# microsoft/XPretrain

Hardware: NVIDIA H100
Metric: video-text pairs/sec (12f x 224^2, 32 tok), CLIP-ViP ViT-B/16 fwd+InfoNCE+bwd (higher is better)
Workload: dtype bf16

## Files before the change

include/xpretrain_b200.h:

```cpp
#ifndef XPRETRAIN_B200_H
#define XPRETRAIN_B200_H

#include <stddef.h>
#include <stdint.h>

#ifdef __cplusplus
extern "C" {
#endif

#define XP_ABI_VERSION 1

int xp_version(void);
const char* xp_last_error(void);
int64_t xp_launch_count(void);
void xp_launch_count_reset(void);

enum { XP_ACT_NONE = 0, XP_ACT_QUICK_GELU = 1, XP_ACT_DQUICK_GELU = 2, XP_ACT_GELU_ERF = 3, XP_ACT_DGELU_ERF = 4 };
enum { XP_OUT_BF16 = 0, XP_OUT_F32 = 1, XP_OUT_F32_ATOMIC = 2 };

typedef struct XpGemm {
  const void* a;
  const void* b;
  void* c;
  const float* bias;
  const void* residual;
  void* aux;
  int64_t M, N, K;
  int64_t lda, ldb, ldc, ldr, ld_aux;
  int32_t a_layout, b_layout;
  int32_t act, out;
  int32_t splits;
  int32_t scale_cols;
  float alpha, col_scale;
  int64_t c_group, c_group_stride, r_group, r_group_stride;
  int32_t block_n;
  int32_t max_ctas;
  int32_t cta_pair;
  int32_t reserved;
} XpGemm;

int xp_gemm(const XpGemm* g, void* stream);

typedef struct XpRowMap {
  int64_t group, group_stride, ld;
  const int64_t* offsets;
} XpRowMap;

int xp_layernorm_fwd(const void* x, const XpRowMap* xmap, void* y, const XpRowMap* ymap, const float* gamma,
// ... 162 lines not shown
```

xpretrain_b200/_lib.py:

```python
from __future__ import annotations

import ctypes as C
import os

_HERE = os.path.dirname(os.path.abspath(__file__))
LIB_PATH = os.path.join(_HERE, "lib", "libxpretrain_b200.so")

c_void_p, c_int, c_i64, c_float = C.c_void_p, C.c_int32, C.c_int64, C.c_float


class XpGemm(C.Structure):
    _fields_ = [
        ("a", c_void_p), ("b", c_void_p), ("c", c_void_p), ("bias", c_void_p), ("residual", c_void_p), ("aux", c_void_p),
        ("M", c_i64), ("N", c_i64), ("K", c_i64),
        ("lda", c_i64), ("ldb", c_i64), ("ldc", c_i64), ("ldr", c_i64), ("ld_aux", c_i64),
        ("a_layout", c_int), ("b_layout", c_int), ("act", c_int), ("out", c_int),
        ("splits", c_int), ("scale_cols", c_int), ("alpha", c_float), ("col_scale", c_float),
        ("c_group", c_i64), ("c_group_stride", c_i64), ("r_group", c_i64), ("r_group_stride", c_i64),
        ("block_n", c_int), ("max_ctas", c_int), ("cta_pair", c_int), ("reserved", c_int),
    ]


class XpRowMap(C.Structure):
    _fields_ = [("group", c_i64), ("group_stride", c_i64), ("ld", c_i64), ("offsets", c_void_p)]
# ... 8 lines not shown

class XpDenseAttn(C.Structure):
    _fields_ = [("n_rows", c_i64), ("ld_qkv", c_i64), ("ld_out", c_i64), ("heads", c_int), ("n_seq", c_int),
                ("seq_len", c_int), ("reserved", c_int)]


class XpNceGather(C.Structure):
    _fields_ = [("vis_local", c_void_p), ("txt_local", c_void_p), ("peer_bufs", c_void_p), ("logit_scale", c_void_p),
                ("g_scaled", c_void_p), ("vis_hi", c_void_p), ("txt_hi", c_void_p), ("loss", c_void_p),
                ("d_logit_scale", c_void_p), ("workspace", c_void_p), ("rank", c_int), ("world", c_int), ("b", c_int),
                ("d", c_int), ("epoch", C.c_uint32), ("mode", c_int), ("ld_g", c_i64)]


class XpNceTerm(C.Structure):
    _fields_ = [("axis", c_int), ("members", c_int), ("excl_diag", c_int), ("target", c_int)]


class XpNceTerms(C.Structure):
    _fields_ = [("z", c_void_p * 3), ("g", c_void_p * 3), ("ld", c_i64 * 3), ("n", c_int * 3), ("n_mats", c_int),
                ("n_terms", c_int), ("term", XpNceTerm * 6), ("logit_scale", c_void_p), ("scale", c_float),
                ("loss", c_void_p), ("d_logit_scale", c_void_p), ("workspace", c_void_p)]


ACT_NONE, ACT_QUICK_GELU, ACT_DQUICK_GELU, ACT_GELU_ERF, ACT_DGELU_ERF = 0, 1, 2, 3, 4
OUT_BF16, OUT_F32, OUT_F32_ATOMIC = 0, 1, 2
DTYPE_F32, DTYPE_BF16, DTYPE_F16 = 0, 1, 2

P = C.POINTER
SIGNATURES = {
    "xp_version": (c_int, []),
    "xp_last_error": (C.c_char_p, []),
    "xp_launch_count": (c_i64, []),
    "xp_launch_count_reset": (None, []),
    "xp_gemm": (c_int, [P(XpGemm), c_void_p]),
    "xp_layernorm_fwd": (c_int, [c_void_p, P(XpRowMap), c_void_p, P(XpRowMap), c_void_p, c_void_p, c_void_p, c_void_p,
                                 c_i64, c_int, c_float, c_void_p]),
    "xp_layernorm_add_fwd": (c_int, [c_void_p, P(XpRowMap), c_int, c_void_p, P(XpRowMap), c_void_p, P(XpRowMap), c_void_p,
                                     P(XpRowMap), c_int, c_void_p, c_void_p, c_void_p, c_void_p, c_i64, c_int, c_float,
                                     c_void_p]),
    "xp_layernorm_bwd": (c_int, [c_void_p, P(XpRowMap), c_void_p, P(XpRowMap), c_int, c_void_p, c_void_p, c_void_p, c_void_p,
                                 P(XpRowMap), c_void_p, P(XpRowMap), c_void_p, c_void_p, c_void_p, c_i64, c_int, c_void_p]),
    "xp_l2norm_fwd": (c_int, [c_void_p, c_void_p, c_void_p, c_int, c_int, c_void_p]),
    "xp_l2norm_bwd": (c_int, [c_void_p, c_void_p, c_void_p, c_void_p, c_int, c_int, c_float, c_void_p]),
    "xp_frame_pool_fwd": (c_int, [c_void_p, c_void_p, c_void_p, c_void_p, c_int, c_int, c_int, c_void_p]),
    "xp_frame_pool_bwd": (c_int, [c_void_p, c_void_p, c_void_p, c_void_p, c_void_p, c_void_p, c_int, c_int, c_int,
                                  c_float, c_void_p]),
    "xp_colsum_bf16": (c_int, [c_void_p, c_i64, c_void_p, c_i64, c_int, c_float, c_void_p]),
    "xp_cast_f32_bf16": (c_int, [c_void_p, c_void_p, c_i64, c_void_p]),
    "xp_vip_patchify": (c_int, [c_void_p, c_int, c_void_p, c_i64, c_int, c_int, c_int, c_void_p]),
    "xp_vip_patchify_u8": (c_int, [c_void_p, c_void_p, c_i64, c_int, c_int, c_int, P(c_float), P(c_float), c_void_p]),
    "xp_vip_embed_tables": (c_int, [c_void_p, c_void_p, c_void_p, c_void_p, c_void_p, c_void_p, c_int, c_int, c_int,
                                    c_int, c_int, c_int, c_void_p]),
    "xp_vip_embed_bwd": (c_int, [c_void_p, c_void_p, c_void_p, c_void_p, c_void_p, c_void_p, c_int, c_int, c_int, c_int,
                                 c_int, c_int, c_void_p]),
    "xp_text_embed_fwd": (c_int, [c_void_p, c_void_p, c_void_p, c_void_p, c_int, c_int, c_int, c_int, c_void_p,
                                  c_void_p]),
    "xp_text_embed_bwd": (c_int, [c_void_p, c_void_p, c_void_p, c_void_p, c_int, c_int, c_int, c_int, c_void_p]),
    "xp_eos_offsets": (c_int, [c_void_p, c_void_p, c_void_p, c_int, c_int, c_int, c_void_p]),
    "xp_vip_attention_workspace_bytes": (c_i64, [c_int, c_int, c_int, c_int]),
    "xp_vip_attention_fwd": (c_int, [c_void_p, c_void_p, c_void_p, c_void_p, c_int, c_int, c_int, c_int, c_int, c_int,
                                     c_void_p]),
    "xp_vip_attention_bwd": (c_int, [c_void_p, c_void_p, c_void_p, c_void_p, c_void_p, c_void_p, c_int, c_int, c_int,
                                     c_int, c_int, c_int, c_float, c_void_p]),
    "xp_text_attention_fwd": (c_int, [c_void_p, c_void_p, c_void_p, c_void_p, c_int, c_int, c_int, c_int, c_void_p]),
    "xp_text_attention_bwd": (c_int, [c_void_p, c_void_p, c_void_p, c_void_p, c_int, c_int, c_int, c_int, c_float,
                                      c_void_p]),
# ... 59 lines not shown
```

xpretrain_b200/csrc/attn_wgmma.cuh:

```cuda
#pragma once
#include "ptx.cuh"
#include "mma_frag.cuh"

namespace xp {

constexpr int ATILE = 64;
constexpr int ATILE_BYTES = ATILE * 128;
constexpr int STREAM_THREADS = 384;

constexpr int stream_fwd_smem(int stages) { return (2 + 2 * stages) * ATILE_BYTES + 1024 + 64; }
constexpr int stream_kv_smem(int stages) { return (4 + 2 * stages) * ATILE_BYTES + stages * 2 * ATILE * 4 + 1024 + 64; }
constexpr int stream_q_smem(int stages) { return (4 + 2 * stages) * ATILE_BYTES + 1024 + 64; }

__device__ __forceinline__ uint64_t kdesc(uint32_t addr) { return make_smem_desc_sw128(addr, 16, 1024); }
__device__ __forceinline__ uint64_t mndesc(uint32_t addr) { return make_smem_desc_sw128(addr, 8192, 1024); }

__device__ __forceinline__ void acc_to_afrag(const float (&x)[32], uint32_t (&a)[4][4]) {
#pragma unroll
  for (int ks = 0; ks < 4; ++ks) {
    a[ks][0] = pack_bf16(x[8 * ks + 0], x[8 * ks + 1]);
    a[ks][1] = pack_bf16(x[8 * ks + 2], x[8 * ks + 3]);
    a[ks][2] = pack_bf16(x[8 * ks + 4], x[8 * ks + 5]);
    a[ks][3] = pack_bf16(x[8 * ks + 6], x[8 * ks + 7]);
  }
// ... 43 lines not shown
  for (int i = 0; i < 32; ++i) {
    const float pv = fast_exp2(fmaf(s[i], LOG2E, -mb[(i >> 1) & 1]));
    s[i] = pv;
    l_run[(i >> 1) & 1] += pv;
  }
  uint32_t ph[4][4], pl[4][4];
  acc_to_afrag(s, ph);
#pragma unroll
  for (int ks = 0; ks < 4; ++ks)
#pragma unroll
    for (int j = 0; j < 4; ++j)
      pl[ks][j] = pack_bf16(s[8 * ks + 2 * j] - bf16_lo(ph[ks][j]), s[8 * ks + 2 * j + 1] - bf16_hi(ph[ks][j]));
  wgmma_fence_regs(o);
  wgmma_fence();
#pragma unroll
  for (int ks = 0; ks < 4; ++ks) {
    const uint64_t vd = mndesc(sV + ks * 16 * 128);
    wgmma_m64n64k16_rs<1>(o, ph[ks], vd);
    wgmma_m64n64k16_rs<1>(o, pl[ks], vd);
  }
  wgmma_commit();
  wgmma_wait<0>();
  wgmma_fence_regs(o);
}

__device__ __forceinline__ void quad_sum(float (&l_run)[2]) {
#pragma unroll
  for (int r = 0; r < 2; ++r) {
    l_run[r] += __shfl_xor_sync(0xffffffffu, l_run[r], 1);
    l_run[r] += __shfl_xor_sync(0xffffffffu, l_run[r], 2);
  }
}

template <class Live>
__device__ __forceinline__ void kv_step(uint32_t sK, uint32_t sV, uint32_t sQ, uint32_t sdO, const float* s_lse,
                                        const float* s_delta, float (&dk)[32], float (&dv)[32], Live live) {
  const int lane = threadIdx.x & 31, k_lo = ((threadIdx.x >> 5) & 3) * 16 + (lane >> 2);
  float st[32], dpt[32];
#pragma unroll
  for (int i = 0; i < 32; ++i) st[i] = dpt[i] = 0.f;
  wgmma_fence_regs(st);
  wgmma_fence_regs(dpt);
  wgmma_fence();
#pragma unroll
  for (int ks = 0; ks < 4; ++ks) {
    wgmma_m64n64k16_ss<0, 0>(st, kdesc(sK + ks * 32), kdesc(sQ + ks * 32));
    wgmma_m64n64k16_ss<0, 0>(dpt, kdesc(sV + ks * 32), kdesc(sdO + ks * 32));
  }
  wgmma_commit();
  wgmma_wait<0>();
  wgmma_fence_regs(st);
  wgmma_fence_regs(dpt);
#pragma unroll
  for (int i = 0; i < 8; ++i)
#pragma unroll
    for (int e = 0; e < 4; ++e) {
      const int q = i * 8 + (lane & 3) * 2 + (e & 1);
      const float p = live(q, k_lo + (e >> 1) * 8) ? fast_exp2(fmaf(st[4 * i + e], LOG2E, -s_lse[q])) : 0.f;
      st[4 * i + e] = p;
      dpt[4 * i + e] = p * (dpt[4 * i + e] - s_delta[q]);
    }
  uint32_t ap[4][4], ad[4][4];
  acc_to_afrag(st, ap);
  acc_to_afrag(dpt, ad);
  wgmma_fence_regs(dv);
  wgmma_fence_regs(dk);
  wgmma_fence();
#pragma unroll
  for (int ks = 0; ks < 4; ++ks) {
    wgmma_m64n64k16_rs<1>(dv, ap[ks], mndesc(sdO + ks * 16 * 128));
    wgmma_m64n64k16_rs<1>(dk, ad[ks], mndesc(sQ + ks * 16 * 128));
  }
  wgmma_commit();
  wgmma_wait<0>();
  wgmma_fence_regs(dv);
  wgmma_fence_regs(dk);
}

template <class Live>
__device__ __forceinline__ void q_step(uint32_t sQ, uint32_t sdO, uint32_t sK, uint32_t sV, const float (&lse_r)[2],
                                       const float (&del_r)[2], float (&dq)[32], Live live) {
  const int lane = threadIdx.x & 31, q_lo = ((threadIdx.x >> 5) & 3) * 16 + (lane >> 2);
  float s[32], dp[32];
#pragma unroll
  for (int i = 0; i < 32; ++i) s[i] = dp[i] = 0.f;
  wgmma_fence_regs(s);
  wgmma_fence_regs(dp);
  wgmma_fence();
#pragma unroll
  for (int ks = 0; ks < 4; ++ks) {
    wgmma_m64n64k16_ss<0, 0>(s, kdesc(sQ + ks * 32), kdesc(sK + ks * 32));
    wgmma_m64n64k16_ss<0, 0>(dp, kdesc(sdO + ks * 32), kdesc(sV + ks * 32));
  }
  wgmma_commit();
  wgmma_wait<0>();
  wgmma_fence_regs(s);
  wgmma_fence_regs(dp);
#pragma unroll
  for (int i = 0; i < 8; ++i)
#pragma unroll
    for (int e = 0; e < 4; ++e) {
      const bool valid = live(q_lo + (e >> 1) * 8, i * 8 + (lane & 3) * 2 + (e & 1));
      const float p = valid ? fast_exp2(fmaf(s[4 * i + e], LOG2E, -lse_r[e >> 1])) : 0.f;
      dp[4 * i + e] = p * (dp[4 * i + e] - del_r[e >> 1]);
    }
  uint32_t ad[4][4];
  acc_to_afrag(dp, ad);
  wgmma_fence_regs(dq);
  wgmma_fence();
#pragma unroll
  for (int ks = 0; ks < 4; ++ks) wgmma_m64n64k16_rs<1>(dq, ad[ks], mndesc(sK + ks * 16 * 128));
  wgmma_commit();
  wgmma_wait<0>();
  wgmma_fence_regs(dq);
}

template <int STAGES>
__device__ __forceinline__ void init_ring(uint64_t* q_full, uint64_t* full, uint64_t* empty, uint32_t full_count,
                                          int nlive, const CUtensorMap* tm0, const CUtensorMap* tm1) {
  if (threadIdx.x == 0) {
    tma_prefetch_desc(tm0);
    tma_prefetch_desc(tm1);
    mbar_init(q_full, 1);
#pragma unroll
    for (int s = 0; s < STAGES; ++s) {
      mbar_init(&full[s], full_count);
      mbar_init(&empty[s], 4 * nlive);
    }
    fence_barrier_init();
  }
  __syncthreads();
}
__device__ __forceinline__ void release_stage(uint64_t* empty, int s) {
  __syncwarp();
  if ((threadIdx.x & 31) == 0) mbar_arrive(&empty[s]);
}

template <class P>
__device__ __forceinline__ void produce_kv_blocks(const P& p, const CUtensorMap* tm, uint8_t* sm, int ring,
                                                  uint64_t* full, uint64_t* empty) {
  for (int kb = 0; kb < p.ntiles(); ++kb) {
    const int s = kb % P::STAGES;
    mbar_wait_nocall(&empty[s], ((kb / P::STAGES) & 1) ^ 1);
    uint8_t* st = sm + (ring + 2 * s) * ATILE_BYTES;
// ... 187 lines not shown
```

xpretrain_b200/csrc/common.cu:

```cuda
#include "common.h"

#include <mutex>

#include "../../include/xpretrain_b200.h"

namespace xp {

static thread_local std::string t_error;
std::atomic<int64_t> g_launches{0};

void set_error(const std::string& msg) { t_error = msg; }
int fail(const std::string& msg) {
  t_error = msg;
  return -1;
}

int sm_count() {
  static int cached[64] = {0};
  int dev = 0;
  if (cudaGetDevice(&dev) != cudaSuccess || dev < 0 || dev >= 64) return 132;
  if (cached[dev] == 0) {
    int n = 0;
    if (cudaDeviceGetAttribute(&n, cudaDevAttrMultiProcessorCount, dev) != cudaSuccess || n <= 0) n = 132;
    cached[dev] = n;
  }
  return cached[dev];
}

typedef CUresult (*EncodeTiledFn)(CUtensorMap*, CUtensorMapDataType, cuuint32_t, void*, const cuuint64_t*,
                                  const cuuint64_t*, const cuuint32_t*, const cuuint32_t*, CUtensorMapInterleave,
                                  CUtensorMapSwizzle, CUtensorMapL2promotion, CUtensorMapFloatOOBfill);

static EncodeTiledFn encode_fn() {
  static EncodeTiledFn fn = nullptr;
  static std::once_flag once;
  std::call_once(once, [] {
    void* p = nullptr;
    cudaDriverEntryPointQueryResult q;
    if (cudaGetDriverEntryPoint("cuTensorMapEncodeTiled", &p, cudaEnableDefault, &q) == cudaSuccess &&
        q == cudaDriverEntryPointSuccess)
      fn = reinterpret_cast<EncodeTiledFn>(p);
  });
  return fn;
}

typedef CUresult (*CtxGetCurrentFn)(CUcontext*);
typedef CUresult (*CtxSetCurrentFn)(CUcontext);
typedef CUresult (*PointerGetAttributeFn)(void*, CUpointer_attribute, CUdeviceptr);

static void* driver_symbol(const char* name) {
  void* p = nullptr;
  cudaDriverEntryPointQueryResult q;
  if (cudaGetDriverEntryPoint(name, &p, cudaEnableDefault, &q) != cudaSuccess || q != cudaDriverEntryPointSuccess)
    return nullptr;
  return p;
}

int ensure_context(const void* device_ptr) {
  static thread_local bool bound = false;
// ... 38 lines not shown
  cuuint32_t estr[2] = {1, 1};
  CUresult r = fn(out, CU_TENSOR_MAP_DATA_TYPE_BFLOAT16, 2, const_cast<void*>(base), dims, strides, box, estr,
                  CU_TENSOR_MAP_INTERLEAVE_NONE, CU_TENSOR_MAP_SWIZZLE_128B, CU_TENSOR_MAP_L2_PROMOTION_L2_256B,
                  CU_TENSOR_MAP_FLOAT_OOB_FILL_NONE);
  if (r != CUDA_SUCCESS) return fail("cuTensorMapEncodeTiled failed with CUresult " + std::to_string(int(r)));
  return 0;
}

int make_tmap_bf16_3d(CUtensorMap* out, const void* base, uint64_t inner, uint64_t mid, uint64_t outer,
                      uint64_t row_stride, uint64_t mid_stride, uint32_t box_inner, uint32_t box_mid) {
  EncodeTiledFn fn = encode_fn();
  if (!fn) return fail("cuTensorMapEncodeTiled unavailable (no CUDA driver / no GPU): this library has no CPU path");
  if ((reinterpret_cast<uintptr_t>(base) & 15) != 0) return fail("tensor map: base pointer must be 16-byte aligned");
  if ((row_stride * 2) % 16 != 0 || (mid_stride * 2) % 16 != 0)
    return fail("tensor map: strides must be multiples of 8 bf16 elements");
  cuuint64_t dims[3] = {inner, mid, outer};
  cuuint64_t strides[2] = {row_stride * 2, mid_stride * 2};
  cuuint32_t box[3] = {box_inner, box_mid, 1};
  cuuint32_t estr[3] = {1, 1, 1};
  CUresult r = fn(out, CU_TENSOR_MAP_DATA_TYPE_BFLOAT16, 3, const_cast<void*>(base), dims, strides, box, estr,
                  CU_TENSOR_MAP_INTERLEAVE_NONE, CU_TENSOR_MAP_SWIZZLE_128B, CU_TENSOR_MAP_L2_PROMOTION_L2_256B,
                  CU_TENSOR_MAP_FLOAT_OOB_FILL_NONE);
  if (r != CUDA_SUCCESS) return fail("cuTensorMapEncodeTiled failed with CUresult " + std::to_string(int(r)));
  return 0;
}

}

extern "C" {
int xp_version(void) { return XP_ABI_VERSION; }
const char* xp_last_error(void) { return xp::t_error.c_str(); }
int64_t xp_launch_count(void) { return xp::g_launches.load(); }
void xp_launch_count_reset(void) { xp::g_launches.store(0); }
}
```

xpretrain_b200/csrc/common.h:

```cpp
#pragma once
#include <cuda.h>
#include <cuda_runtime.h>
#include <stdint.h>

#include <atomic>
#include <string>

namespace xp {

void set_error(const std::string& msg);
int fail(const std::string& msg);
extern std::atomic<int64_t> g_launches;
inline void count_launch(int n = 1) { g_launches.fetch_add(n, std::memory_order_relaxed); }

int sm_count();

int make_tmap_bf16_2d(CUtensorMap* out, const void* base, uint64_t inner, uint64_t outer, uint64_t row_stride,
                      uint32_t box_inner, uint32_t box_outer);
int make_tmap_bf16_3d(CUtensorMap* out, const void* base, uint64_t inner, uint64_t mid, uint64_t outer,
                      uint64_t row_stride, uint64_t mid_stride, uint32_t box_inner, uint32_t box_mid);

int ensure_context(const void* device_ptr);
#define XP_ENTER(ptr)                                   \
  do {                                                  \
    if (::xp::ensure_context(ptr) != 0) return -1;      \
  } while (0)

#define XP_CHECK_CUDA(expr)                                                                         \
  do {                                                                                              \
    cudaError_t _e = (expr);                                                                        \
    if (_e != cudaSuccess) return ::xp::fail(std::string(#expr) + ": " + cudaGetErrorString(_e)); \
  } while (0)

#define XP_CHECK_LAUNCH(name)                                                                             \
  do {                                                                                                    \
    cudaError_t _e = cudaGetLastError();                                                                  \
    if (_e != cudaSuccess) return ::xp::fail(std::string(name) + " launch: " + cudaGetErrorString(_e)); \
    ::xp::count_launch();                                                                                 \
  } while (0)

}
```

xpretrain_b200/csrc/vip_attention.cu:

```cuda
#include "../../include/xpretrain_b200.h"
#include "common.h"
#include "attn_wgmma.cuh"
#include "vip_attention.h"

namespace xp {

constexpr int SROWS = 256;
constexpr int GROW = 248;
constexpr int MAT_BYTES = SROWS * 128;
constexpr int TILE_BYTES = 64 * 128;
constexpr int ATT_THREADS = 256;

__device__ __forceinline__ bool row_valid(int r, const AttnDims& d) { return r < d.L || (r >= GROW && r < GROW + d.M); }
__device__ __forceinline__ bool row_global(int r) { return r >= GROW; }
__device__ __forceinline__ int row_seq(int r, const AttnDims& d) { return r >= GROW ? r - GROW : d.M + r; }
__device__ __forceinline__ bool tile_live(int k, const AttnDims& d) { return k == 3 || 64 * k < d.L; }

template <int NMAT>
__device__ __forceinline__ void stage_rows(uint8_t* sm, uint64_t* bar, const CUtensorMap* const (&mapL)[NMAT],
                                           const CUtensorMap* const (&mapM)[NMAT], const int (&col)[NMAT], const AttnDims& d,
                                           int b, int t) {
  if (threadIdx.x == 0) {
    mbar_init(bar, 1);
    fence_barrier_init();
  }
  const uint32_t base = smem_u32(sm);
  for (int idx = threadIdx.x; idx < NMAT * SROWS * 8; idx += ATT_THREADS) {
    const int m = idx / (SROWS * 8), row = (idx >> 3) % SROWS;
    if (!row_valid(row, d)) st_shared_zero16(base + m * MAT_BYTES + row * 128 + (idx & 7) * 16);
  }
  fence_proxy_async_smem();
  __syncthreads();
  if (threadIdx.x == 0) {
    mbar_arrive_expect_tx(bar, NMAT * (d.L + d.M) * 128);
#pragma unroll
    for (int m = 0; m < NMAT; ++m) {
// ... 57 lines not shown
        const long long tr = token_row(d, b, t, row_seq(row, d));
        __nv_bfloat16* dst = out + tr * d.ld_o + h * HD + (lane & 3) * 2;
#pragma unroll
        for (int i = 0; i < 8; ++i)
          *reinterpret_cast<uint32_t*>(dst + i * 8) = pack_bf16(o[4 * i + 2 * r] * inv, o[4 * i + 2 * r + 1] * inv);
        if ((lane & 3) == 0)
          lse[(static_cast<long long>(b) * d.H + h) * d.S + (tr - static_cast<long long>(b) * d.S)] = m_run[r] + logf(l_run[r]);
      }
    }
  }
}

__global__ void __launch_bounds__(64)
vip_attn_fwd_combine_kernel(const float* __restrict__ part, __nv_bfloat16* __restrict__ out, float* __restrict__ lse,
                            const AttnDims d) {
  const int h = blockIdx.x, b = blockIdx.y, c = threadIdx.x;
  for (int m = 0; m < d.M; ++m) {
    const float* p0 = part + ((static_cast<long long>(b) * d.H + h) * d.T * d.M + m) * 66;
    float mx = -INFINITY;
    for (int t = 0; t < d.T; ++t) mx = fmaxf(mx, p0[static_cast<long long>(t) * d.M * 66]);
    float l = 0.f, acc = 0.f;
    for (int t = 0; t < d.T; ++t) {
      const float* p = p0 + static_cast<long long>(t) * d.M * 66;
      const float w = __expf(p[0] - mx);
      l += p[1] * w;
      acc += p[2 + c] * w;
    }
    out[(static_cast<long long>(b) * d.S + m) * d.ld_o + h * HD + c] = __float2bfloat16(acc / l);
    if (c == 0) lse[(static_cast<long long>(b) * d.H + h) * d.S + m] = mx + logf(l);
  }
}


__global__ void __launch_bounds__(ATT_THREADS, 1)
vip_attn_bwd_kernel(const __grid_constant__ CUtensorMap tmL, const __grid_constant__ CUtensorMap tmM,
                    const __grid_constant__ CUtensorMap tdL, const __grid_constant__ CUtensorMap tdM,
                    const __nv_bfloat16* __restrict__ out, const __nv_bfloat16* __restrict__ dout, const float* __restrict__ lse,
                    __nv_bfloat16* __restrict__ dqkv, float* __restrict__ gpart, const AttnDims d, float q_scale) {
  extern __shared__ uint8_t smem_raw[];
  uint8_t* sm = smem_raw + (((smem_u32(smem_raw) + 1023u) & ~1023u) - smem_u32(smem_raw));
  float* s_lse = reinterpret_cast<float*>(sm + 4 * MAT_BYTES);
  float* s_delta = s_lse + SROWS;
  uint64_t* bar = reinterpret_cast<uint64_t*>(s_delta + SROWS);
  const int t = blockIdx.x, h = blockIdx.y, b = blockIdx.z;
  {
    const CUtensorMap* const mL[4] = {&tmL, &tmL, &tmL, &tdL};
    const CUtensorMap* const mM[4] = {&tmM, &tmM, &tmM, &tdM};
    const int col[4] = {h * HD, d.C + h * HD, 2 * d.C + h * HD, h * HD};
    stage_rows<4>(sm, bar, mL, mM, col, d, b, t);
  }
  for (int base = 0; base < SROWS; base += ATT_THREADS / 8) {
    const int row = base + (threadIdx.x >> 3), chunk = threadIdx.x & 7;
    float dot = 0.f;
    const bool valid = row_valid(row, d);
    long long tr = 0;
    if (valid) {
      tr = token_row(d, b, t, row_seq(row, d));
      const long long off = tr * d.ld_o + h * HD + chunk * 8;
      const uint4 g = *reinterpret_cast<const uint4*>(dout + off);
      const uint4 o = *reinterpret_cast<const uint4*>(out + off);
      const uint32_t gw[4] = {g.x, g.y, g.z, g.w}, ow[4] = {o.x, o.y, o.z, o.w};
#pragma unroll
      for (int i = 0; i < 4; ++i) dot += bf16_lo(gw[i]) * bf16_lo(ow[i]) + bf16_hi(gw[i]) * bf16_hi(ow[i]);
    }
    dot += __shfl_xor_sync(0xffffffffu, dot, 1);
    dot += __shfl_xor_sync(0xffffffffu, dot, 2);
    dot += __shfl_xor_sync(0xffffffffu, dot, 4);
    if (chunk == 0) {
      s_delta[row] = dot;
      s_lse[row] = valid ? lse[(static_cast<long long>(b) * d.H + h) * d.S + (tr - static_cast<long long>(b) * d.S)] * LOG2E
                         : INFINITY;
    }
  }
  __syncthreads();

  const uint32_t sQ = smem_u32(sm), sK = sQ + MAT_BYTES, sV = sK + MAT_BYTES, sdO = sV + MAT_BYTES;
  const int wg = threadIdx.x >> 7, wq = (threadIdx.x >> 5) & 3, lane = threadIdx.x & 31;
  const bool mask_gg = (t != 0);
  const auto pair_live = [&](int q, int key) {
    return row_valid(q, d) && row_valid(key, d) && !(mask_gg && row_global(q) && row_global(key));
  };
  float* gp = gpart + ((static_cast<long long>(b) * d.H + h) * d.T + t) * d.M * 3 * HD;

  for (int kt = wg; kt < 4; kt += 2) {
    if (!tile_live(kt, d)) continue;
    const int k_lo = kt * 64 + wq * 16 + (lane >> 2);
    float dk[32], dv[32];
#pragma unroll
    for (int i = 0; i < 32; ++i) dk[i] = dv[i] = 0.f;
#pragma unroll 1
    for (int qb = 0; qb < 4; ++qb) {
      if (!tile_live(qb, d)) continue;
      kv_step(sK + kt * TILE_BYTES, sV + kt * TILE_BYTES, sQ + qb * TILE_BYTES, sdO + qb * TILE_BYTES, s_lse + qb * 64,
              s_delta + qb * 64, dk, dv, [&](int q, int key) { return pair_live(qb * 64 + q, kt * 64 + key); });
    }
#pragma unroll
    for (int r = 0; r < 2; ++r) {
      const int key = k_lo + r * 8;
      if (!row_valid(key, d)) continue;
      if (!row_global(key)) {
        __nv_bfloat16* row = dqkv + token_row(d, b, t, row_seq(key, d)) * d.ld_qkv + h * HD + (lane & 3) * 2;
#pragma unroll
        for (int i = 0; i < 8; ++i) {
          *reinterpret_cast<uint32_t*>(row + d.C + i * 8) = pack_bf16(dk[4 * i + 2 * r], dk[4 * i + 2 * r + 1]);
          *reinterpret_cast<uint32_t*>(row + 2 * d.C + i * 8) = pack_bf16(dv[4 * i + 2 * r], dv[4 * i + 2 * r + 1]);
        }
      } else {
        float* g = gp + static_cast<long long>(key - GROW) * 3 * HD + (lane & 3) * 2;
#pragma unroll
        for (int i = 0; i < 8; ++i) {
          g[HD + i * 8] = dk[4 * i + 2 * r]; g[HD + i * 8 + 1] = dk[4 * i + 2 * r + 1];
          g[2 * HD + i * 8] = dv[4 * i + 2 * r]; g[2 * HD + i * 8 + 1] = dv[4 * i + 2 * r + 1];
        }
      }
    }
  }

  for (int qt = wg; qt < 4; qt += 2) {
    if (!tile_live(qt, d)) continue;
    const int q_lo = qt * 64 + wq * 16 + (lane >> 2);
    const float lse_r[2] = {s_lse[q_lo], s_lse[q_lo + 8]}, del_r[2] = {s_delta[q_lo], s_delta[q_lo + 8]};
    float dq[32];
#pragma unroll
    for (int i = 0; i < 32; ++i) dq[i] = 0.f;
#pragma unroll 1
    for (int kb = 0; kb < 4; ++kb) {
      if (!tile_live(kb, d)) continue;
      q_step(sQ + qt * TILE_BYTES, sdO + qt * TILE_BYTES, sK + kb * TILE_BYTES, sV + kb * TILE_BYTES, lse_r, del_r, dq,
             [&](int q, int key) { return pair_live(qt * 64 + q, kb * 64 + key); });
    }
#pragma unroll
    for (int r = 0; r < 2; ++r) {
      const int q = q_lo + r * 8;
      if (!row_valid(q, d)) continue;
      if (!row_global(q)) {
        __nv_bfloat16* row = dqkv + token_row(d, b, t, row_seq(q, d)) * d.ld_qkv + h * HD + (lane & 3) * 2;
#pragma unroll
        for (int i = 0; i < 8; ++i)
          *reinterpret_cast<uint32_t*>(row + i * 8) = pack_bf16(dq[4 * i + 2 * r] * q_scale, dq[4 * i + 2 * r + 1] * q_scale);
      } else {
        float* g = gp + static_cast<long long>(q - GROW) * 3 * HD + (lane & 3) * 2;
#pragma unroll
        for (int i = 0; i < 8; ++i) {
          g[i * 8] = dq[4 * i + 2 * r];
          g[i * 8 + 1] = dq[4 * i + 2 * r + 1];
        }
      }
    }
  }
}

__global__ void __launch_bounds__(192)
vip_attn_bwd_combine_kernel(const float* __restrict__ gpart, __nv_bfloat16* __restrict__ dqkv, const AttnDims d,
                            float q_scale) {
  const int h = blockIdx.x, b = blockIdx.y;
  const int which = threadIdx.x / HD, c = threadIdx.x % HD;
  for (int m = 0; m < d.M; ++m) {
    float acc = 0.f;
    for (int t = 0; t < d.T; ++t)
      acc += gpart[((((static_cast<long long>(b) * d.H + h) * d.T + t) * d.M + m) * 3 + which) * HD + c];
    if (which == 0) acc *= q_scale;
    dqkv[(static_cast<long long>(b) * d.S + m) * d.ld_qkv + static_cast<long long>(which) * d.C + h * HD + c] =
        __float2bfloat16(acc);
  }
}


static int make_dims(AttnDims& d, int B, int H, int T, int L, int M, int C) {
  if (C != H * HD) return fail("vip_attention: head_dim must be 64 (C == 64*H)");
  if (L < 1) return fail("vip_attention: L must be >= 1");
  if (M < 1 || M > 8) return fail("vip_attention: 1 <= M <= 8 global tokens");
  d.B = B; d.H = H; d.T = T; d.L = L; d.M = M;
  d.S = static_cast<long long>(M) + static_cast<long long>(T) * L;
  d.C = C;
  d.ld_qkv = 3LL * C;
  d.ld_o = C;
  return 0;
}

static int make_row_maps(CUtensorMap* mL, CUtensorMap* mM, const void* base, long long width, const AttnDims& d) {
  const uint64_t rows = static_cast<uint64_t>(d.B) * static_cast<uint64_t>(d.S);
  if (make_tmap_bf16_2d(mL, base, width, rows, width, HD, d.L)) return -1;
  return make_tmap_bf16_2d(mM, base, width, rows, width, HD, d.M);
}

constexpr int FWD_SMEM = 3 * MAT_BYTES + 1024 + 64;
constexpr int BWD_SMEM = 4 * MAT_BYTES + 2 * SROWS * 4 + 1024 + 64;

}

using namespace xp;

extern "C" int64_t xp_vip_attention_workspace_bytes(int32_t B, int32_t H, int32_t T, int32_t M) {
  return static_cast<int64_t>(B) * H * T * M * 3 * HD * sizeof(float);
}

extern "C" int xp_vip_attention_fwd(const void* qkv, void* out, float* lse, float* workspace, int32_t B, int32_t H,
                                    int32_t T, int32_t L, int32_t M, int32_t C, void* stream) {
  XP_ENTER(qkv);
  AttnDims d;
  if (make_dims(d, B, H, T, L, M, C)) return -1;
  cudaStream_t st = static_cast<cudaStream_t>(stream);
  if (M + L > VIP_STAGED_MAX_ROWS) {
    if (vip_long_attn_fwd(d, qkv, out, lse, workspace, st)) return -1;
  } else {
    CUtensorMap mL, mM;
    if (make_row_maps(&mL, &mM, qkv, 3LL * C, d)) return -1;
    static bool attr = false;
    if (!attr) {
      XP_CHECK_CUDA(cudaFuncSetAttribute(vip_attn_fwd_kernel, cudaFuncAttributeMaxDynamicSharedMemorySize, FWD_SMEM));
      attr = true;
    }
    vip_attn_fwd_kernel<<<dim3(T, H, B), ATT_THREADS, FWD_SMEM, st>>>(mL, mM, static_cast<__nv_bfloat16*>(out), lse, workspace, d);
    XP_CHECK_LAUNCH("vip_attn_fwd_kernel");
  }
  vip_attn_fwd_combine_kernel<<<dim3(H, B), 64, 0, st>>>(workspace, static_cast<__nv_bfloat16*>(out), lse, d);
  XP_CHECK_LAUNCH("vip_attn_fwd_combine_kernel");
  return 0;
}

extern "C" int xp_vip_attention_bwd(const void* qkv, const void* out, const void* dout, const float* lse, void* dqkv,
                                    float* workspace, int32_t B, int32_t H, int32_t T, int32_t L, int32_t M, int32_t C,
                                    float q_scale, void* stream) {
  XP_ENTER(qkv);
  AttnDims d;
  if (make_dims(d, B, H, T, L, M, C)) return -1;
  cudaStream_t st = static_cast<cudaStream_t>(stream);
  if (M + L > VIP_STAGED_MAX_ROWS) {
    if (vip_long_attn_bwd(d, qkv, out, dout, lse, dqkv, workspace, q_scale, st)) return -1;
  } else {
    CUtensorMap mL, mM, gL, gM;
    if (make_row_maps(&mL, &mM, qkv, 3LL * C, d) || make_row_maps(&gL, &gM, dout, C, d)) return -1;
    static bool attr = false;
    if (!attr) {
      XP_CHECK_CUDA(cudaFuncSetAttribute(vip_attn_bwd_kernel, cudaFuncAttributeMaxDynamicSharedMemorySize, BWD_SMEM));
      attr = true;
    }
    vip_attn_bwd_kernel<<<dim3(T, H, B), ATT_THREADS, BWD_SMEM, st>>>(
        mL, mM, gL, gM, static_cast<const __nv_bfloat16*>(out), static_cast<const __nv_bfloat16*>(dout), lse,
        static_cast<__nv_bfloat16*>(dqkv), workspace, d, q_scale);
    XP_CHECK_LAUNCH("vip_attn_bwd_kernel");
  }
  vip_attn_bwd_combine_kernel<<<dim3(H, B), 192, 0, st>>>(workspace, static_cast<__nv_bfloat16*>(dqkv), d, q_scale);
  XP_CHECK_LAUNCH("vip_attn_bwd_combine_kernel");
  return 0;
}
```

xpretrain_b200/csrc/vip_attention.h:

```cpp
#pragma once
#include <cuda_runtime.h>

namespace xp {

constexpr int VIP_STAGED_MAX_ROWS = 208;

struct AttnDims {
  int B, H, T, L, M;
  long long S;
  long long ld_qkv;
  long long ld_o;
  int C;
};

__device__ __forceinline__ long long token_row(const AttnDims& d, int b, int t, int i) {
  return static_cast<long long>(b) * d.S + (i < d.M ? i : d.M + static_cast<long long>(t) * d.L + (i - d.M));
}

int vip_long_attn_fwd(const AttnDims& d, const void* qkv, void* out, float* lse, float* part, cudaStream_t st);
int vip_long_attn_bwd(const AttnDims& d, const void* qkv, const void* out, const void* dout, const float* lse, void* dqkv,
                      float* gpart, float q_scale, cudaStream_t st);

}
```

xpretrain_b200/ops.py:

```python
from __future__ import annotations

import ctypes as C
from typing import Optional

import torch

from . import _lib
from ._lib import XpDenseAttn, XpGemm, XpRowMap, XpSegAttn, check, lib

bf16, f32 = torch.bfloat16, torch.float32


def _stream() -> int:
    return torch.cuda.current_stream().cuda_stream


def _p(t: Optional[torch.Tensor]):
    if t is None:
        return None
    if not t.is_cuda:
        raise _lib.XpError("xpretrain_b200 kernels need CUDA tensors (there is no CPU path)")
    return t.data_ptr()


# ... 14 lines not shown
    assert a.dtype == bf16 and b.dtype == bf16
    if bias is not None:
        assert bias.dtype == f32 and bias.is_contiguous()
    g = XpGemm()
    g.a = _p(a) + a_offset * 2
    g.b = _p(b) + b_offset * 2
    g.c = _p(out) + c_offset * out.element_size()
    g.bias = _p(bias)
    g.residual = _p(residual)
    g.aux = _p(aux)
    g.M, g.N, g.K = M, N, K
    g.lda, g.ldb, g.ldc, g.ldr, g.ld_aux = lda, ldb, ldc, ldr, ld_aux
    g.a_layout, g.b_layout, g.act, g.out = a_layout, b_layout, act, out_mode
    g.splits, g.scale_cols, g.alpha, g.col_scale = splits, scale_cols, alpha, col_scale
    g.c_group, g.c_group_stride, g.r_group, g.r_group_stride = c_group, c_group_stride, r_group, r_group_stride
    g.block_n, g.max_ctas = block_n, _sm_limit
    if _gemm_timer is None:
        check(lib().xp_gemm(C.byref(g), _stream()), "xp_gemm")
    else:
        e0, e1 = torch.cuda.Event(enable_timing=True), torch.cuda.Event(enable_timing=True)
        e0.record()
        check(lib().xp_gemm(C.byref(g), _stream()), "xp_gemm")
        e1.record()
        _gemm_timer.append((2.0 * M * N * K, e0, e1))


_gemm_timer = None
_sm_limit = 0


def set_sm_limit(n: int) -> None:
    global _sm_limit
    _sm_limit = max(0, int(n))


def set_gemm_timer(records) -> None:
    global _gemm_timer
    _gemm_timer = records


def linear_fwd(x: torch.Tensor, w: torch.Tensor, bias: Optional[torch.Tensor], out: torch.Tensor, **kw) -> None:
    M, K = x.shape
    N = w.shape[0]
    gemm(x, w, out, M=M, N=N, K=K, lda=x.stride(0), ldb=w.stride(0), ldc=out.stride(0), bias=bias, **kw)


def linear_dgrad(dy: torch.Tensor, w: torch.Tensor, dx: torch.Tensor, **kw) -> None:
    M, N = dy.shape
    K = w.shape[1]
    gemm(dy, w, dx, M=M, N=K, K=N, lda=dy.stride(0), ldb=w.stride(0), ldc=dx.stride(0), b_layout=1, **kw)


def wgrad_plan(n_out: int, n_in: int, rows: int, sms: int = 0):
    sms = sms or _sm_limit or 132
    bn = 256 if n_in >= 256 else 128
    tiles, slots = ((n_out + 127) // 128) * ((n_in + bn - 1) // bn), sms
    best, best_eff = 1, 0.0
    for s in range(1, 33):
        if s > 1 and rows // s < 1024:
            break
        total = tiles * s
        eff = total / (((total + slots - 1) // slots) * slots)
        if eff > best_eff + 0.02:
            best, best_eff = s, eff
    return bn, best

# ... 312 lines not shown
```

Before: 293.9.

## Make ViP attention backward persistent with warp-specialized TMA double-buffered pipeline

The staged attention backward kernel becomes a persistent kernel over (b,h,t) items. A producer warpgroup loads Q/K/V/dO with TMA into two slots and computes the lse and delta row stats from the staged dO, while two consumer warpgroups compute dK/dV and dQ. Rows are packed tightly (frame rows padded to a multiple of 8, then global rows) and the last tile uses fewer k-steps. This cuts padded MMA work and hides load and stat latency behind compute, at the cost of more shared memory, register rebalancing and more complex barrier logic. It also adds an SM-limit setter so the grid size can be capped.

```diff
diff --git a/include/xpretrain_b200.h b/include/xpretrain_b200.h
--- a/include/xpretrain_b200.h
+++ b/include/xpretrain_b200.h
@@ -14,6 +14,7 @@
 const char* xp_last_error(void);
 int64_t xp_launch_count(void);
 void xp_launch_count_reset(void);
+void xp_set_sm_limit(int32_t n);
 
 enum { XP_ACT_NONE = 0, XP_ACT_QUICK_GELU = 1, XP_ACT_DQUICK_GELU = 2, XP_ACT_GELU_ERF = 3, XP_ACT_DGELU_ERF = 4 };
 enum { XP_OUT_BF16 = 0, XP_OUT_F32 = 1, XP_OUT_F32_ATOMIC = 2 };
diff --git a/xpretrain_b200/_lib.py b/xpretrain_b200/_lib.py
--- a/xpretrain_b200/_lib.py
+++ b/xpretrain_b200/_lib.py
@@ -64,6 +64,7 @@
     "xp_last_error": (C.c_char_p, []),
     "xp_launch_count": (c_i64, []),
     "xp_launch_count_reset": (None, []),
+    "xp_set_sm_limit": (None, [c_int]),
     "xp_gemm": (c_int, [P(XpGemm), c_void_p]),
     "xp_layernorm_fwd": (c_int, [c_void_p, P(XpRowMap), c_void_p, P(XpRowMap), c_void_p, c_void_p, c_void_p, c_void_p,
                                  c_i64, c_int, c_float, c_void_p]),
diff --git a/xpretrain_b200/csrc/attn_wgmma.cuh b/xpretrain_b200/csrc/attn_wgmma.cuh
--- a/xpretrain_b200/csrc/attn_wgmma.cuh
+++ b/xpretrain_b200/csrc/attn_wgmma.cuh
@@ -99,7 +99,7 @@
   }
 }
 
-template <class Live>
+template <int NKS = 4, class Live>
 __device__ __forceinline__ void kv_step(uint32_t sK, uint32_t sV, uint32_t sQ, uint32_t sdO, const float* s_lse,
                                         const float* s_delta, float (&dk)[32], float (&dv)[32], Live live) {
   const int lane = threadIdx.x & 31, k_lo = ((threadIdx.x >> 5) & 3) * 16 + (lane >> 2);
@@ -134,7 +134,7 @@
   wgmma_fence_regs(dk);
   wgmma_fence();
 #pragma unroll
-  for (int ks = 0; ks < 4; ++ks) {
+  for (int ks = 0; ks < NKS; ++ks) {
     wgmma_m64n64k16_rs<1>(dv, ap[ks], mndesc(sdO + ks * 16 * 128));
     wgmma_m64n64k16_rs<1>(dk, ad[ks], mndesc(sQ + ks * 16 * 128));
   }
@@ -144,7 +144,7 @@
   wgmma_fence_regs(dk);
 }
 
-template <class Live>
+template <int NKS = 4, class Live>
 __device__ __forceinline__ void q_step(uint32_t sQ, uint32_t sdO, uint32_t sK, uint32_t sV, const float (&lse_r)[2],
                                        const float (&del_r)[2], float (&dq)[32], Live live) {
   const int lane = threadIdx.x & 31, q_lo = ((threadIdx.x >> 5) & 3) * 16 + (lane >> 2);
@@ -176,7 +176,7 @@
   wgmma_fence_regs(dq);
   wgmma_fence();
 #pragma unroll
-  for (int ks = 0; ks < 4; ++ks) wgmma_m64n64k16_rs<1>(dq, ad[ks], mndesc(sK + ks * 16 * 128));
+  for (int ks = 0; ks < NKS; ++ks) wgmma_m64n64k16_rs<1>(dq, ad[ks], mndesc(sK + ks * 16 * 128));
   wgmma_commit();
   wgmma_wait<0>();
   wgmma_fence_regs(dq);
diff --git a/xpretrain_b200/csrc/common.cu b/xpretrain_b200/csrc/common.cu
--- a/xpretrain_b200/csrc/common.cu
+++ b/xpretrain_b200/csrc/common.cu
@@ -25,6 +25,13 @@
     cached[dev] = n;
   }
   return cached[dev];
+}
+
+static std::atomic<int> g_sm_limit{0};
+
+int sm_limit() {
+  const int n = sm_count(), cap = g_sm_limit.load(std::memory_order_relaxed);
+  return cap > 0 && cap < n ? cap : n;
 }
 
 typedef CUresult (*EncodeTiledFn)(CUtensorMap*, CUtensorMapDataType, cuuint32_t, void*, const cuuint64_t*,
@@ -129,4 +136,5 @@
 const char* xp_last_error(void) { return xp::t_error.c_str(); }
 int64_t xp_launch_count(void) { return xp::g_launches.load(); }
 void xp_launch_count_reset(void) { xp::g_launches.store(0); }
+void xp_set_sm_limit(int32_t n) { xp::g_sm_limit.store(n > 0 ? n : 0); }
 }
diff --git a/xpretrain_b200/csrc/common.h b/xpretrain_b200/csrc/common.h
--- a/xpretrain_b200/csrc/common.h
+++ b/xpretrain_b200/csrc/common.h
@@ -14,6 +14,7 @@
 inline void count_launch(int n = 1) { g_launches.fetch_add(n, std::memory_order_relaxed); }
 
 int sm_count();
+int sm_limit();
 
 int make_tmap_bf16_2d(CUtensorMap* out, const void* base, uint64_t inner, uint64_t outer, uint64_t row_stride,
                       uint32_t box_inner, uint32_t box_outer);
diff --git a/xpretrain_b200/csrc/vip_attention.cu b/xpretrain_b200/csrc/vip_attention.cu
--- a/xpretrain_b200/csrc/vip_attention.cu
+++ b/xpretrain_b200/csrc/vip_attention.cu
@@ -2,6 +2,8 @@
 #include "common.h"
 #include "attn_wgmma.cuh"
 #include "vip_attention.h"
+
+#include <type_traits>
 
 namespace xp {
 
@@ -125,121 +127,213 @@
 }
 
 
-__global__ void __launch_bounds__(ATT_THREADS, 1)
+constexpr int PROWS = VIP_STAGED_MAX_ROWS;
+constexpr int PMAT_BYTES = PROWS * 128;
+constexpr int BWD_SLOT_BYTES = 4 * PMAT_BYTES;
+constexpr int OVERREACH = (4 * 64 - PROWS) * 128;
+constexpr int BWD_STAT_BYTES = 2 * 2 * 256 * 4;
+constexpr int BWD_HEAD_BYTES = BWD_STAT_BYTES + 1024;
+constexpr int BWD_THREADS = 384;
+static_assert(PMAT_BYTES % 1024 == 0, "packed matrices must stay 1024-byte aligned for the 128B swizzle");
+
+__device__ __forceinline__ int packed_g(int L) { return (L + 7) & ~7; }
+
+template <class F>
+__device__ __forceinline__ void with_ksteps(int n, F f) {
+  switch (n) {
+    case 1: f(std::integral_constant<int, 1>()); break;
+    case 2: f(std::integral_constant<int, 2>()); break;
+    case 3: f(std::integral_constant<int, 3>()); break;
+    default: f(std::integral_constant<int, 4>()); break;
+  }
+}
+
+__device__ __forceinline__ bool prow_valid(int r, int L, int G, int M) { return r < L || (r >= G && r < G + M); }
+
+__global__ void __launch_bounds__(BWD_THREADS, 1)
 vip_attn_bwd_kernel(const __grid_constant__ CUtensorMap tmL, const __grid_constant__ CUtensorMap tmM,
                     const __grid_constant__ CUtensorMap tdL, const __grid_constant__ CUtensorMap tdM,
-                    const __nv_bfloat16* __restrict__ out, const __nv_bfloat16* __restrict__ dout, const float* __restrict__ lse,
+                    const __nv_bfloat16* __restrict__ out, const float* __restrict__ lse,
                     __nv_bfloat16* __restrict__ dqkv, float* __restrict__ gpart, const AttnDims d, float q_scale) {
   extern __shared__ uint8_t smem_raw[];
   uint8_t* sm = smem_raw + (((smem_u32(smem_raw) + 1023u) & ~1023u) - smem_u32(smem_raw));
-  float* s_lse = reinterpret_cast<float*>(sm + 4 * MAT_BYTES);
-  float* s_delta = s_lse + SROWS;
-  uint64_t* bar = reinterpret_cast<uint64_t*>(s_delta + SROWS);
-  const int t = blockIdx.x, h = blockIdx.y, b = blockIdx.z;
+  float* s_stat = reinterpret_cast<float*>(sm);
+  uint64_t* full = reinterpret_cast<uint64_t*>(sm + BWD_STAT_BYTES);
+  uint64_t* stat = full + 2;
+  uint64_t* empty = stat + 2;
+  uint8_t* slots = sm + BWD_HEAD_BYTES;
+  const int L = d.L, M = d.M, G = packed_g(L), R = (G + M + 15) & ~15, nt = (R + 63) / 64;
+  const int nitems = d.B * d.H * d.T;
+  const int wg = threadIdx.x >> 7;
+
+  if (threadIdx.x == 0) {
+    tma_prefetch_desc(&tmL);
+    tma_prefetch_desc(&tmM);
+    tma_prefetch_desc(&tdL);
+    tma_prefetch_desc(&tdM);
+    for (int s = 0; s < 2; ++s) {
+      mbar_init(&full[s], 1);
+      mbar_init(&stat[s], 128);
+      mbar_init(&empty[s], 8);
+    }
+    fence_barrier_init();
+  }
   {
-    const CUtensorMap* const mL[4] = {&tmL, &tmL, &tmL, &tdL};
-    const CUtensorMap* const mM[4] = {&tmM, &tmM, &tmM, &tdM};
-    const int col[4] = {h * HD, d.C + h * HD, 2 * d.C + h * HD, h * HD};
-    stage_rows<4>(sm, bar, mL, mM, col, d, b, t);
-  }
-  for (int base = 0; base < SROWS; base += ATT_THREADS / 8) {
-    const int row = base + (threadIdx.x >> 3), chunk = threadIdx.x & 7;
-    float dot = 0.f;
-    const bool valid = row_valid(row, d);
-    long long tr = 0;
-    if (valid) {
-      tr = token_row(d, b, t, row_seq(row, d));
-      const long long off = tr * d.ld_o + h * HD + chunk * 8;
-      const uint4 g = *reinterpret_cast<const uint4*>(dout + off);
-      const uint4 o = *reinterpret_cast<const uint4*>(out + off);
-      const uint32_t gw[4] = {g.x, g.y, g.z, g.w}, ow[4] = {o.x, o.y, o.z, o.w};
-#pragma unroll
-      for (int i = 0; i < 4; ++i) dot += bf16_lo(gw[i]) * bf16_lo(ow[i]) + bf16_hi(gw[i]) * bf16_hi(ow[i]);
-    }
-    dot += __shfl_xor_sync(0xffffffffu, dot, 1);
-    dot += __shfl_xor_sync(0xffffffffu, dot, 2);
-    dot += __shfl_xor_sync(0xffffffffu, dot, 4);
-    if (chunk == 0) {
-      s_delta[row] = dot;
-      s_lse[row] = valid ? lse[(static_cast<long long>(b) * d.H + h) * d.S + (tr - static_cast<long long>(b) * d.S)] * LOG2E
-                         : INFINITY;
-    }
-  }
+    const uint32_t base = smem_u32(slots);
+    for (int idx = threadIdx.x; idx < 2 * 4 * PROWS * 8; idx += BWD_THREADS) {
+      const int mat = idx / (PROWS * 8), row = (idx >> 3) % PROWS;
+      if (row < R && !prow_valid(row, L, G, M)) st_shared_zero16(base + mat * PMAT_BYTES + row * 128 + (idx & 7) * 16);
+    }
+  }
+  fence_proxy_async_smem();
   __syncthreads();
 
-  const uint32_t sQ = smem_u32(sm), sK = sQ + MAT_BYTES, sV = sK + MAT_BYTES, sdO = sV + MAT_BYTES;
-  const int wg = threadIdx.x >> 7, wq = (threadIdx.x >> 5) & 3, lane = threadIdx.x & 31;
-  const bool mask_gg = (t != 0);
-  const auto pair_live = [&](int q, int key) {
-    return row_valid(q, d) && row_valid(key, d) && !(mask_gg && row_global(q) && row_global(key));
-  };
-  float* gp = gpart + ((static_cast<long long>(b) * d.H + h) * d.T + t) * d.M * 3 * HD;
-
-  for (int kt = wg; kt < 4; kt += 2) {
-    if (!tile_live(kt, d)) continue;
-    const int k_lo = kt * 64 + wq * 16 + (lane >> 2);
-    float dk[32], dv[32];
-#pragma unroll
-    for (int i = 0; i < 32; ++i) dk[i] = dv[i] = 0.f;
-#pragma unroll 1
-    for (int qb = 0; qb < 4; ++qb) {
-      if (!tile_live(qb, d)) continue;
-      kv_step(sK + kt * TILE_BYTES, sV + kt * TILE_BYTES, sQ + qb * TILE_BYTES, sdO + qb * TILE_BYTES, s_lse + qb * 64,
-              s_delta + qb * 64, dk, dv, [&](int q, int key) { return pair_live(qb * 64 + q, kt * 64 + key); });
-    }
-#pragma unroll
-    for (int r = 0; r < 2; ++r) {
-      const int key = k_lo + r * 8;
-      if (!row_valid(key, d)) continue;
-      if (!row_global(key)) {
-        __nv_bfloat16* row = dqkv + token_row(d, b, t, row_seq(key, d)) * d.ld_qkv + h * HD + (lane & 3) * 2;
-#pragma unroll
-        for (int i = 0; i < 8; ++i) {
-          *reinterpret_cast<uint32_t*>(row + d.C + i * 8) = pack_bf16(dk[4 * i + 2 * r], dk[4 * i + 2 * r + 1]);
-          *reinterpret_cast<uint32_t*>(row + 2 * d.C + i * 8) = pack_bf16(dv[4 * i + 2 * r], dv[4 * i + 2 * r + 1]);
-        }
-      } else {
-        float* g = gp + static_cast<long long>(key - GROW) * 3 * HD + (lane & 3) * 2;
-#pragma unroll
-        for (int i = 0; i < 8; ++i) {
-          g[HD + i * 8] = dk[4 * i + 2 * r]; g[HD + i * 8 + 1] = dk[4 * i + 2 * r + 1];
-          g[2 * HD + i * 8] = dv[4 * i + 2 * r]; g[2 * HD + i * 8 + 1] = dv[4 * i + 2 * r + 1];
+  if (wg == 0) {
+    setmaxnreg_dec<40>();
+    const int tid = threadIdx.x;
+    int k = 0;
+    for (int item = blockIdx.x; item < nitems; item += gridDim.x, ++k) {
+      const int s = k & 1;
+      const uint32_t ph = (k >> 1) & 1;
+      const int t = item % d.T, bh = item / d.T, h = bh % d.H, b = bh / d.H;
+      uint8_t* slot = slots + s * BWD_SLOT_BYTES;
+      mbar_wait_nocall(&empty[s], ph ^ 1);
+      if (tid == 0) {
+        const CUtensorMap* const mL[4] = {&tmL, &tmL, &tmL, &tdL};
+        const CUtensorMap* const mM[4] = {&tmM, &tmM, &tmM, &tdM};
+        const int col[4] = {h * HD, d.C + h * HD, 2 * d.C + h * HD, h * HD};
+        mbar_arrive_expect_tx(&full[s], 4 * (L + M) * 128);
+#pragma unroll
+        for (int m = 0; m < 4; ++m) {
+          tma_load_2d(slot + m * PMAT_BYTES, mL[m], &full[s], col[m],
+                      static_cast<int>(b * d.S + M + static_cast<long long>(t) * L));
+          tma_load_2d(slot + m * PMAT_BYTES + G * 128, mM[m], &full[s], col[m], static_cast<int>(b * d.S));
         }
       }
-    }
-  }
-
-  for (int qt = wg; qt < 4; qt += 2) {
-    if (!tile_live(qt, d)) continue;
-    const int q_lo = qt * 64 + wq * 16 + (lane >> 2);
-    const float lse_r[2] = {s_lse[q_lo], s_lse[q_lo + 8]}, del_r[2] = {s_delta[q_lo], s_delta[q_lo + 8]};
-    float dq[32];
-#pragma unroll
-    for (int i = 0; i < 32; ++i) dq[i] = 0.f;
-#pragma unroll 1
-    for (int kb = 0; kb < 4; ++kb) {
-      if (!tile_live(kb, d)) continue;
-      q_step(sQ + qt * TILE_BYTES, sdO + qt * TILE_BYTES, sK + kb * TILE_BYTES, sV + kb * TILE_BYTES, lse_r, del_r, dq,
-             [&](int q, int key) { return pair_live(qt * 64 + q, kb * 64 + key); });
-    }
-#pragma unroll
-    for (int r = 0; r < 2; ++r) {
-      const int q = q_lo + r * 8;
-      if (!row_valid(q, d)) continue;
-      if (!row_global(q)) {
-        __nv_bfloat16* row = dqkv + token_row(d, b, t, row_seq(q, d)) * d.ld_qkv + h * HD + (lane & 3) * 2;
-#pragma unroll
-        for (int i = 0; i < 8; ++i)
-          *reinterpret_cast<uint32_t*>(row + i * 8) = pack_bf16(dq[4 * i + 2 * r] * q_scale, dq[4 * i + 2 * r + 1] * q_scale);
-      } else {
-        float* g = gp + static_cast<long long>(q - GROW) * 3 * HD + (lane & 3) * 2;
-#pragma unroll
-        for (int i = 0; i < 8; ++i) {
-          g[i * 8] = dq[4 * i + 2 * r];
-          g[i * 8 + 1] = dq[4 * i + 2 * r + 1];
+      mbar_wait_nocall(&full[s], ph);
+      const uint8_t* sdo = slot + 3 * PMAT_BYTES;
+      float* st = s_stat + s * 512;
+      const int half = tid & 1;
+#pragma unroll 1
+      for (int row = tid >> 1; row < 256; row += 64) {
+        const bool valid = prow_valid(row, L, G, M);
+        float dot = 0.f;
+        long long tr = 0;
+        if (valid) {
+          tr = token_row(d, b, t, row < L ? M + row : row - G);
+          const __nv_bfloat16* o = out + tr * d.ld_o + h * HD + half * 32;
+#pragma unroll
+          for (int j = 0; j < 4; ++j) {
+            const int c = half * 4 + j;
+            const uint4 g = *reinterpret_cast<const uint4*>(sdo + row * 128 + ((c ^ (row & 7)) << 4));
+            const uint4 ov = *reinterpret_cast<const uint4*>(o + 8 * j);
+            const uint32_t gw[4] = {g.x, g.y, g.z, g.w}, ow[4] = {ov.x, ov.y, ov.z, ov.w};
+#pragma unroll
+            for (int i = 0; i < 4; ++i) dot += bf16_lo(gw[i]) * bf16_lo(ow[i]) + bf16_hi(gw[i]) * bf16_hi(ow[i]);
+          }
+        }
+        dot += __shfl_xor_sync(0xffffffffu, dot, 1);
+        if (half == 0) {
+          st[row] = valid ? lse[static_cast<long long>(bh) * d.S + (tr - static_cast<long long>(b) * d.S)] * LOG2E
+                          : INFINITY;
+          st[256 + row] = dot;
         }
       }
-    }
+      mbar_arrive(&stat[s]);
+    }
+    return;
+  }
+
+  setmaxnreg_inc<232>();
+  const int c = wg - 1, wq = (threadIdx.x >> 5) & 3, lane = threadIdx.x & 31;
+  const auto nks = [&](int blk) { return (R - 64 * blk) / 16; };
+  int k = 0;
+#pragma unroll 1
+  for (int item = blockIdx.x; item < nitems; item += gridDim.x, ++k) {
+    const int s = k & 1;
+    const uint32_t ph = (k >> 1) & 1;
+    const int t = item % d.T, bh = item / d.T, h = bh % d.H, b = bh / d.H;
+    const uint32_t sQ = smem_u32(slots + s * BWD_SLOT_BYTES), sK = sQ + PMAT_BYTES, sV = sK + PMAT_BYTES,
+                   sdO = sV + PMAT_BYTES;
+    const float* s_lse = s_stat + s * 512;
+    const float* s_delta = s_lse + 256;
+    const bool mask_gg = (t != 0);
+    const auto pair_live = [&](int q, int key) {
+      return prow_valid(q, L, G, M) && prow_valid(key, L, G, M) && !(mask_gg && q >= G && key >= G);
+    };
+    float* gp = gpart + (static_cast<long long>(bh) * d.T + t) * M * 3 * HD;
+    mbar_wait_nocall(&full[s], ph);
+    mbar_wait_nocall(&stat[s], ph);
+
+#pragma unroll 1
+    for (int kt = c; kt < nt; kt += 2) {
+      const int k_lo = kt * 64 + wq * 16 + (lane >> 2);
+      float dk[32], dv[32];
+#pragma unroll
+      for (int i = 0; i < 32; ++i) dk[i] = dv[i] = 0.f;
+#pragma unroll 1
+      for (int qb = 0; qb < nt; ++qb)
+        with_ksteps(nks(qb), [&](auto n) {
+          kv_step<decltype(n)::value>(sK + kt * TILE_BYTES, sV + kt * TILE_BYTES, sQ + qb * TILE_BYTES,
+                                      sdO + qb * TILE_BYTES, s_lse + qb * 64, s_delta + qb * 64, dk, dv,
+                                      [&](int q, int key) { return pair_live(qb * 64 + q, kt * 64 + key); });
+        });
+#pragma unroll
+      for (int r = 0; r < 2; ++r) {
+        const int key = k_lo + r * 8;
+        if (!prow_valid(key, L, G, M)) continue;
+        if (key < L) {
+          __nv_bfloat16* row = dqkv + token_row(d, b, t, M + key) * d.ld_qkv + h * HD + (lane & 3) * 2;
+#pragma unroll
+          for (int i = 0; i < 8; ++i) {
+            *reinterpret_cast<uint32_t*>(row + d.C + i * 8) = pack_bf16(dk[4 * i + 2 * r], dk[4 * i + 2 * r + 1]);
+            *reinterpret_cast<uint32_t*>(row + 2 * d.C + i * 8) = pack_bf16(dv[4 * i + 2 * r], dv[4 * i + 2 * r + 1]);
+          }
+        } else {
+          float* g = gp + static_cast<long long>(key - G) * 3 * HD + (lane & 3) * 2;
+#pragma unroll
+          for (int i = 0; i < 8; ++i) {
+            g[HD + i * 8] = dk[4 * i + 2 * r]; g[HD + i * 8 + 1] = dk[4 * i + 2 * r + 1];
+            g[2 * HD + i * 8] = dv[4 * i + 2 * r]; g[2 * HD + i * 8 + 1] = dv[4 * i + 2 * r + 1];
+          }
+        }
+      }
+    }
+
+#pragma unroll 1
+    for (int qt = c; qt < nt; qt += 2) {
+      const int q_lo = qt * 64 + wq * 16 + (lane >> 2);
+      const float lse_r[2] = {s_lse[q_lo], s_lse[q_lo + 8]}, del_r[2] = {s_delta[q_lo], s_delta[q_lo + 8]};
+      float dq[32];
+#pragma unroll
+      for (int i = 0; i < 32; ++i) dq[i] = 0.f;
+#pragma unroll 1
+      for (int kb = 0; kb < nt; ++kb)
+        with_ksteps(nks(kb), [&](auto n) {
+          q_step<decltype(n)::value>(sQ + qt * TILE_BYTES, sdO + qt * TILE_BYTES, sK + kb * TILE_BYTES,
+                                     sV + kb * TILE_BYTES, lse_r, del_r, dq,
+                                     [&](int q, int key) { return pair_live(qt * 64 + q, kb * 64 + key); });
+        });
+#pragma unroll
+      for (int r = 0; r < 2; ++r) {
+        const int q = q_lo + r * 8;
+        if (!prow_valid(q, L, G, M)) continue;
+        if (q < L) {
+          __nv_bfloat16* row = dqkv + token_row(d, b, t, M + q) * d.ld_qkv + h * HD + (lane & 3) * 2;
+#pragma unroll
+          for (int i = 0; i < 8; ++i)
+            *reinterpret_cast<uint32_t*>(row + i * 8) = pack_bf16(dq[4 * i + 2 * r] * q_scale, dq[4 * i + 2 * r + 1] * q_scale);
+        } else {
+          float* g = gp + static_cast<long long>(q - G) * 3 * HD + (lane & 3) * 2;
+#pragma unroll
+          for (int i = 0; i < 8; ++i) {
+            g[i * 8] = dq[4 * i + 2 * r];
+            g[i * 8 + 1] = dq[4 * i + 2 * r + 1];
+          }
+        }
+      }
+    }
+    release_stage(empty, s);
   }
 }
 
@@ -278,7 +372,8 @@
 }
 
 constexpr int FWD_SMEM = 3 * MAT_BYTES + 1024 + 64;
-constexpr int BWD_SMEM = 4 * MAT_BYTES + 2 * SROWS * 4 + 1024 + 64;
+constexpr int BWD_SMEM = BWD_HEAD_BYTES + 2 * BWD_SLOT_BYTES + OVERREACH + 1024;
+static_assert(BWD_SMEM <= 227 * 1024, "backward stage exceeds the opt-in shared memory of an SM");
 
 }
 
@@ -319,9 +414,11 @@
   AttnDims d;
   if (make_dims(d, B, H, T, L, M, C)) return -1;
   cudaStream_t st = static_cast<cudaStream_t>(stream);
-  if (M + L > VIP_STAGED_MAX_ROWS) {
+  if (vip_packed_rows(L, M) > VIP_STAGED_MAX_ROWS) {
     if (vip_long_attn_bwd(d, qkv, out, dout, lse, dqkv, workspace, q_scale, st)) return -1;
   } else {
+    const long long items = static_cast<long long>(B) * H * T;
+    if (items > 0x7fffffffLL) return fail("vip_attention: B*H*T must fit in int32");
     CUtensorMap mL, mM, gL, gM;
     if (make_row_maps(&mL, &mM, qkv, 3LL * C, d) || make_row_maps(&gL, &gM, dout, C, d)) return -1;
     static bool attr = false;
@@ -329,9 +426,9 @@
       XP_CHECK_CUDA(cudaFuncSetAttribute(vip_attn_bwd_kernel, cudaFuncAttributeMaxDynamicSharedMemorySize, BWD_SMEM));
       attr = true;
     }
-    vip_attn_bwd_kernel<<<dim3(T, H, B), ATT_THREADS, BWD_SMEM, st>>>(
-        mL, mM, gL, gM, static_cast<const __nv_bfloat16*>(out), static_cast<const __nv_bfloat16*>(dout), lse,
-        static_cast<__nv_bfloat16*>(dqkv), workspace, d, q_scale);
+    const int grid = static_cast<int>(items < sm_limit() ? items : sm_limit());
+    vip_attn_bwd_kernel<<<grid, BWD_THREADS, BWD_SMEM, st>>>(mL, mM, gL, gM, static_cast<const __nv_bfloat16*>(out), lse,
+                                                             static_cast<__nv_bfloat16*>(dqkv), workspace, d, q_scale);
     XP_CHECK_LAUNCH("vip_attn_bwd_kernel");
   }
   vip_attn_bwd_combine_kernel<<<dim3(H, B), 192, 0, st>>>(workspace, static_cast<__nv_bfloat16*>(dqkv), d, q_scale);
diff --git a/xpretrain_b200/csrc/vip_attention.h b/xpretrain_b200/csrc/vip_attention.h
--- a/xpretrain_b200/csrc/vip_attention.h
+++ b/xpretrain_b200/csrc/vip_attention.h
@@ -4,6 +4,7 @@
 namespace xp {
 
 constexpr int VIP_STAGED_MAX_ROWS = 208;
+inline int vip_packed_rows(int L, int M) { return (((L + 7) & ~7) + M + 15) & ~15; }
 
 struct AttnDims {
   int B, H, T, L, M;
diff --git a/xpretrain_b200/ops.py b/xpretrain_b200/ops.py
--- a/xpretrain_b200/ops.py
+++ b/xpretrain_b200/ops.py
@@ -70,6 +70,7 @@
 def set_sm_limit(n: int) -> None:
     global _sm_limit
     _sm_limit = max(0, int(n))
+    lib().xp_set_sm_limit(_sm_limit)
 
 
 def set_gemm_timer(records) -> None:
```

New measurement: 303.7, median of 6. +3.3%, better.
